# lisvulaczo/lodestar

Hardware: AMD Instinct MI355X
Metric: BLS signature sets verified/sec (whole node) at 1/2/4/8 MI355X; p50 batch latency (higher is better)
Workload: dtype u32

## Files before the change

### include/lodestar_bls.h

```cpp
#ifndef LODESTAR_BLS_H
#define LODESTAR_BLS_H

#include <stddef.h>
#include <stdint.h>

#ifdef __cplusplus
extern "C" {
#endif

#define LSG_OK 0
#define LSG_ERR_INVALID_ARG 1
#define LSG_ERR_NO_DEVICE 2
#define LSG_ERR_DEVICE 3
#define LSG_ERR_NOMEM 4
#define LSG_ERR_CLOSED 5
#define LSG_ERR_BUSY 6
#define LSG_ERR_ENTROPY 7

#define LSG_BLST_SUCCESS 0
#define LSG_BLST_BAD_ENCODING 1
#define LSG_BLST_POINT_NOT_ON_CURVE 2
#define LSG_BLST_POINT_NOT_IN_GROUP 3
#define LSG_BLST_AGGR_TYPE_MISMATCH 4
#define LSG_BLST_VERIFY_FAIL 5
// ... 144 lines not shown
int lsg_verify_deposits(lsg_ctx* ctx, const uint8_t* data184, size_t n, const uint8_t* domain32, uint64_t seed,
                        uint8_t* valid, int32_t* err);

int lsg_sign(lsg_ctx* ctx, const uint8_t* sks32, const uint8_t* msgs, uint32_t msg_len, size_t n, uint8_t* out96);
int lsg_sk_to_pk(lsg_ctx* ctx, const uint8_t* sks32, size_t n, uint8_t* out96);

int lsg_check_fp2_mul(lsg_ctx* ctx, const uint32_t* in, size_t n, uint32_t* out);
int lsg_check_fp_sqr(lsg_ctx* ctx, const uint32_t* in, size_t n, uint32_t* out);
int lsg_check_fp2_sqr(lsg_ctx* ctx, const uint32_t* in, size_t n, uint32_t* out);
int lsg_check_sums(lsg_ctx* ctx, const uint32_t* in, size_t n, uint32_t* out);
int lsg_check_fp2_lanes(lsg_ctx* ctx, const uint32_t* in, size_t n, uint32_t* out);
int lsg_check_g2_lanes(lsg_ctx* ctx, const uint32_t* in, size_t n, uint32_t* out);
int lsg_check_mf_lanes(lsg_ctx* ctx, const uint32_t* in, size_t n, uint32_t* out);
int lsg_check_pow_lanes(lsg_ctx* ctx, int32_t id, const uint32_t* in, size_t n, uint32_t* out);
int lsg_check_pow_pair(lsg_ctx* ctx, int32_t id, const uint32_t* in, size_t n, uint32_t* out);
int lsg_check_canon(lsg_ctx* ctx, const uint32_t* in, size_t n, const uint8_t* bytes48, size_t nb, uint32_t* out,
                    uint32_t* out_limbs);
int lsg_check_fp2_roots(lsg_ctx* ctx, const uint32_t* in, size_t n, uint32_t* out);
int lsg_check_batch_inv(lsg_ctx* ctx, const uint32_t* in, size_t n, uint32_t* out);
int lsg_check_map_uniform(lsg_ctx* ctx, const uint8_t* ub256, size_t n, uint8_t* out192);
int lsg_check_batch_partial_rnd(lsg_ctx* ctx, const lsg_set* sets, size_t n_sets,
                                const uint64_t* rnd , uint8_t* out576,
                                int32_t* set_err, int32_t* any_error);

int lsg_probe_fp_mul_rate(lsg_ctx* ctx, double* fp_mul_per_s, double* mad_per_s);

int lsg_probe_mad_peak(lsg_ctx* ctx, double* mad_per_s);

int lsg_last_kernel_times(lsg_ctx* ctx, const char** names, double* ms, int max);

// ... 5 lines not shown
```

### lodestar_amd/_native.py

```python
import ctypes
import os
import struct
import threading

HERE = os.path.dirname(os.path.abspath(__file__))
LIB_PATH = os.environ.get("LSG_LIB", os.path.join(HERE, "liblodestar_bls.so"))
AB_LIB_PATH = os.path.join(HERE, "liblodestar_bls_ab.so")

LSG_OK = 0
LSG_ERR_INVALID_ARG = 1
LSG_ERR_NO_DEVICE = 2
LSG_ERR_BUSY = 6
LSG_ERR_ENTROPY = 7

LSG_INVALID = 0
LSG_VALID = 1
LSG_ERROR = 2

LSG_JOB_BATCHABLE = 1
LSG_JOB_PRIORITY = 2
LSG_JOB_VALIDATE_KEYS = 4

BLST_NAMES = {
    0: "BLST_SUCCESS", 1: "BLST_BAD_ENCODING", 2: "BLST_POINT_NOT_ON_CURVE", 3: "BLST_POINT_NOT_IN_GROUP",
# ... 145 lines not shown
_lib_lock = threading.Lock()

EXPORTS = [
    "lsg_init", "lsg_init_devices", "lsg_destroy", "lsg_device_count", "lsg_last_error", "lsg_device_name",
    "lsg_reserve", "lsg_allocation_count", "lsg_verify_jobs", "lsg_verify_sets",
    "lsg_aggregate_pubkeys", "lsg_hash_to_g2", "lsg_sig_decode", "lsg_batch_partial", "lsg_final_verify",
    "lsg_probe_fp_mul_rate", "lsg_last_kernel_times", "lsg_sign", "lsg_sk_to_pk",
    "lsg_submit_jobs", "lsg_wait_jobs", "lsg_wait_jobs_node", "lsg_jobs_partial", "lsg_assign_jobs", "lsg_poll",
    "lsg_final_submit", "lsg_final_wait", "lsg_pipeline_slots", "lsg_probe_mad_peak",
    "lsg_pubkey_table_set", "lsg_pubkey_table_size", "lsg_pubkey_validate",
    "lsg_final_submit_groups", "lsg_final_wait_groups", "lsg_aggregate_signatures",
    "lsg_signing_roots", "lsg_attestation_signing_roots", "lsg_jobs_partial_device", "lsg_final_submit_device",
    "lsg_set_coalesce", "lsg_aggregate_pubkeys_multi", "lsg_check_fp2_mul",
    "lsg_check_fp_sqr", "lsg_check_fp2_sqr", "lsg_check_sums", "lsg_check_fp2_lanes", "lsg_check_g2_lanes", "lsg_check_mf_lanes",
    "lsg_check_canon", "lsg_check_fp2_roots", "lsg_check_batch_inv", "lsg_check_map_uniform",
    "lsg_check_batch_partial_rnd", "lsg_check_pow_lanes", "lsg_check_pow_pair",
    "lsg_deposit_signing_roots", "lsg_verify_deposits",
    "lsg_committees_set", "lsg_committees_clear", "lsg_committee_count",
    "lsg_object_signing_roots", "lsg_object_signing_roots_var",
    "lsg_submit_jobs_grouped", "lsg_wait_jobs_grouped",
    "lsg_msg_cache_set", "lsg_msg_cache_clear", "lsg_msg_cache_get_stats",
]


def load_library(path=LIB_PATH):
    global _lib
    with _lib_lock:
        if _lib is not None and path == LIB_PATH:
            return _lib
        if not os.path.exists(path):
            raise NativeUnavailable(f"{path} not built (run python -c 'import __graft_entry__; __graft_entry__.build()')")
# ... 56 lines not shown
        lib.lsg_aggregate_signatures.argtypes = [vp, ctypes.c_char_p, u32, ctypes.POINTER(u32), sz,
                                                 ctypes.c_char_p, pi32]
        lib.lsg_final_submit.argtypes = [vp, ctypes.c_char_p, sz, pu64]
        lib.lsg_final_wait.argtypes = [vp, u64, pi32]
        lib.lsg_pipeline_slots.argtypes = [vp, pi32]
        lib.lsg_set_coalesce.argtypes = [vp, u32, i32]
        lib.lsg_check_fp2_mul.argtypes = [vp, ctypes.c_char_p, sz, ctypes.c_char_p]
        lib.lsg_check_fp_sqr.argtypes = [vp, ctypes.c_char_p, sz, ctypes.c_char_p]
        lib.lsg_check_fp2_sqr.argtypes = [vp, ctypes.c_char_p, sz, ctypes.c_char_p]
        lib.lsg_check_sums.argtypes = [vp, ctypes.c_char_p, sz, ctypes.c_char_p]
        lib.lsg_check_fp2_lanes.argtypes = [vp, ctypes.c_char_p, sz, ctypes.c_char_p]
        lib.lsg_check_g2_lanes.argtypes = [vp, ctypes.c_char_p, sz, ctypes.c_char_p]
        lib.lsg_check_mf_lanes.argtypes = [vp, ctypes.c_char_p, sz, ctypes.c_char_p]
        lib.lsg_check_pow_lanes.argtypes = [vp, i32, ctypes.c_char_p, sz, ctypes.c_char_p]
        lib.lsg_check_pow_pair.argtypes = [vp, i32, ctypes.c_char_p, sz, ctypes.c_char_p]
        lib.lsg_check_canon.argtypes = [vp, ctypes.c_char_p, sz, ctypes.c_char_p, sz, ctypes.c_char_p, ctypes.c_char_p]
        lib.lsg_check_fp2_roots.argtypes = [vp, ctypes.c_char_p, sz, ctypes.c_char_p]
        lib.lsg_check_batch_inv.argtypes = [vp, ctypes.c_char_p, sz, ctypes.c_char_p]
        lib.lsg_check_map_uniform.argtypes = [vp, ctypes.c_char_p, sz, ctypes.c_char_p]
        lib.lsg_check_batch_partial_rnd.argtypes = [vp, ctypes.POINTER(LsgSet), sz, ctypes.POINTER(u64),
                                                    ctypes.c_char_p, pi32, pi32]
        lib.lsg_probe_mad_peak.argtypes = [vp, ctypes.POINTER(ctypes.c_double)]
        for name in EXPORTS:
            if name != "lsg_last_error":
                getattr(lib, name).restype = ctypes.c_int
        if path == LIB_PATH:
            _lib = lib
        return lib


# ... 549 lines not shown
    def check_g2_lanes(self, words):
        return self._check_lanes("lsg_check_g2_lanes", words)

    def check_mf_lanes(self, words):
        return self._check_lanes("lsg_check_mf_lanes", words)

    def check_pow(self, pow_id, words, lanes=True):
        n = len(words) // 14
        assert len(words) == 14 * n
        fn = "lsg_check_pow_lanes" if lanes else "lsg_check_pow_pair"
        out = ctypes.create_string_buffer(4 * 14 * max(n, 1))
        src = struct.pack(f"<{len(words)}I", *words)
        self._check(getattr(self.lib, fn)(self.h, pow_id, src, n, out), fn)
        return list(struct.unpack(f"<{14 * n}I", out.raw[:4 * 14 * n]))

    def check_canon(self, words, strings=()):
        n, nb = len(words) // 14, len(strings)
        assert len(words) == 14 * n and all(len(b) == 48 for b in strings)
        out = ctypes.create_string_buffer(4 * 54 * max(n, 1))
        limbs = ctypes.create_string_buffer(4 * 14 * max(nb, 1))
        src = struct.pack(f"<{len(words)}I", *words)
        self._check(self.lib.lsg_check_canon(self.h, src, n, b"".join(strings), nb, out, limbs), "lsg_check_canon")
        return (list(struct.unpack(f"<{54 * n}I", out.raw[:4 * 54 * n])),
                list(struct.unpack(f"<{14 * nb}I", limbs.raw[:4 * 14 * nb])))

    def check_fp2_roots(self, words):
        n = len(words) // 28
        assert len(words) == 28 * n
        out = ctypes.create_string_buffer(4 * 58 * n)
        src = struct.pack(f"<{len(words)}I", *words)
# ... 38 lines not shown
```

### lodestar_amd/csrc/lsg_ab.h

```cpp
#pragma once
#include <stdlib.h>

#define LSG_POW_LANES_DEFAULT 1
#define LSG_POW_LANES_MIN_DEFAULT 65536

#ifdef LSG_AB
static inline long lsg_ab_long(const char* name, long dflt) {
  const char* e = getenv(name);
  return e ? atol(e) : dflt;
}
#else
#define lsg_ab_long(name, dflt) ((long)(dflt))
#endif
```

### lodestar_amd/csrc/lsg_curve.hpp

```cpp
#pragma once
#include "lsg_tower.hpp"

LSG_INL fp_t fadd(const fp_t& a, const fp_t& b) { return fp_add(a, b); }
LSG_INL fp2_t fadd(const fp2_t& a, const fp2_t& b) { return fp2_add(a, b); }
LSG_INL fp_t fsub(const fp_t& a, const fp_t& b) { return fp_sub(a, b); }
LSG_INL fp2_t fsub(const fp2_t& a, const fp2_t& b) { return fp2_sub(a, b); }
LSG_INL fp_t fmul(const fp_t& a, const fp_t& b) { return fp_mul(a, b); }
LSG_INL fp2_t fmul(const fp2_t& a, const fp2_t& b) { return fp2_mul(a, b); }
LSG_INL fp_t fsqr(const fp_t& a) { return fp_sqr(a); }
LSG_INL fp2_t fsqr(const fp2_t& a) { return fp2_sqr(a); }
LSG_INL fp_t fneg(const fp_t& a) { return fp_neg(a); }
LSG_INL fp2_t fneg(const fp2_t& a) { return fp2_neg(a); }
LSG_INL fps_t<1, 0> fsum(const fp_t& a) { return fps(a); }
LSG_INL fp2s_t<1, 0> fsum(const fp2_t& a) { return fp2s(a); }
template <int K, int P, int N>
LSG_INL fps_t<K * P, K * N> fsum_mulk(const fps_t<P, N>& a) { return fps_mulk<K>(a); }
template <int K, int P0, int N0, int P1, int N1>
LSG_INL fp2s_t<K * P0, K * N0, K * P1, K * N1> fsum_mulk(const fp2s_t<P0, N0, P1, N1>& a) { return fp2s_mulk<K>(a); }
template <int K> LSG_INL fp_t fmulk(const fp_t& a) { return fp_mulk<K>(a); }
template <int K> LSG_INL fp2_t fmulk(const fp2_t& a) { return fp2_mulk<K>(a); }
template <class F> LSG_INL F fsub2(const F& a, const F& b, const F& c) { return (fsum(a) - b - c).carry(); }
LSG_INL fp_t fmul_b3(const fp_t& a) { return fp_mul12(a); }
LSG_INL fp2_t fmul_b3(const fp2_t& a) { return fp2_mul_b3(a); }
template <int P0, int N0, int P1, int N1>
// ... 174 lines not shown
#endif
LSG_INL const g2p_t& g2_to_pair(const g2p_t& p) { return p; }
template <class F> struct g2_layout;
template <> struct g2_layout<fp2_t> {
  static LSG_INL g2a_t in(const g2a_t& a) { return a; }
};
#ifdef LSG_FP2_LANES
template <> struct g2_layout<fp2v_t> {
  static LSG_INL g2va_t in(const g2a_t& a) { return g2v_from_pair(a); }
};
typedef fp2v_t chain_fp2_t;
#else
typedef fp2_t chain_fp2_t;
#endif

template <class F>
struct jac_t {
  F X, Y, Z;
};

template <class F>
LSG_INL jac_t<F> jac_from_proj(const proj_t<F>& p) {
  F zz = fsqr(p.Z);
  jac_t<F> r;
  bool inf = fis_zero(p.Z);
  r.X = fselect(inf, fone<F>(), fmul(p.X, p.Z));
  r.Y = fselect(inf, fone<F>(), fmul(p.Y, zz));
  r.Z = p.Z;
  return r;
}
// ... 374 lines not shown
```

### lodestar_amd/csrc/lsg_host.hip

```cpp
#include <hip/hip_runtime.h>
#include <rccl/rccl.h>
#include <stdio.h>
#include <stdlib.h>
#include <errno.h>
#include <string.h>
#include <sys/random.h>
#include <time.h>

#include <algorithm>
#include <atomic>
#include <condition_variable>
#include <chrono>
#include <mutex>
#include <shared_mutex>
#include <thread>
#include <unordered_map>
#include <string>
#include <vector>

#include "../../include/lodestar_bls.h"
#include "lsg_launch.h"
#include "lsg_layout.h"
#include "lsg_slp.h"
#include "lsg_ab.h"
// ... 473 lines not shown
}

bool agg_tree_on() { return lsg_ab_long("LSG_AGG_TREE", 0) != 0; }

Switches read_switches() {
  Switches w;
  w.package_group = lsg_ab_long("LSG_PACKAGE_GROUP", 1) != 0;
  w.sub_groups = lsg_ab_long("LSG_SUB_GROUPS", 1) != 0;
  w.nb_merge = lsg_ab_long("LSG_NB_MERGE", 1) != 0;
  w.msg_agg = lsg_ab_long("LSG_MSG_AGG", 1) != 0;
  w.msm_min_group = (size_t)std::max(1L, lsg_ab_long("LSG_MSM_MIN_GROUP", 256));
  w.b0_min = (size_t)std::max(0L, lsg_ab_long("LSG_B0_MIN", 64));
  w.b0_run = (size_t)std::max(2L, lsg_ab_long("LSG_B0_RUN", 4));
  w.seg_fold_wide = (int)lsg_ab_long("LSG_SEG_FOLD_WIDE", SEG_FOLD_WIDE);
  w.slp_items = slp_items_max();
  return w;
}
SegPlan slot_seg(Slot* s, int op, const std::vector<int32_t>& seg_off, const std::vector<int32_t>& seg_len, bool has_idx,
                 size_t idx_off, int32_t dst_base) {
  return plan_seg(s->plan, op, seg_off, seg_len, has_idx, idx_off, dst_base,
                  (int)lsg_ab_long("LSG_SEG_FOLD_WIDE", SEG_FOLD_WIDE));
}

void binv_sizes(size_t n, size_t* lv, size_t* iv);
size_t binv_lv_words(size_t n) {
  size_t a, b;
  binv_sizes(n, &a, &b);
  return a;
}
size_t binv_iv_words(size_t n) {
// ... 361 lines not shown
                                                P_<uint8_t>(s->d_hinf), P_<int32_t>(s->d_seterr), P_<uint32_t>(s->d_H),
                                                fall));
    else
      KL(s, "k_miller_fused_pair",
         lsgk::miller_fused(S_(s), ni, items, items + ni, P_<uint32_t>(s->d_P), P_<uint8_t>(s->d_pinf),
                            P_<uint8_t>(s->d_hinf), P_<int32_t>(s->d_seterr), P_<uint32_t>(s->d_H), fall, true));
    return LSG_OK;
  }
  KL(s, "k_miller_accum",
     lsgk::miller_accum(S_(s), s->K, ni, items, items + ni, P_<uint32_t>(s->d_P), P_<uint8_t>(s->d_pinf),
                        P_<uint8_t>(s->d_hinf), P_<int32_t>(s->d_seterr), (int)s->n_sets, P_<uint32_t>(s->d_lines),
                        fall));
  return LSG_OK;
}

int launch_phase(Slot* s, const PhasePlan& Ph, const uint32_t* rs, uint32_t* fall, bool export_blobs,
                 const uint32_t* rs_msm = nullptr) {
  if (!rs_msm) rs_msm = rs;
  const size_t ng = Ph.groups.size();
  if (ng == 0) return LSG_OK;
  LSG_RC(size_state(s, s->n_sets, s->n_pks, ng, Ph.n_msm, 2));
  s->cur = 1;
  if (Ph.n_msm) {
    LSG_RC(run_seg(s, 1, "msm_buckets", Ph.buckets, rs_msm, P_<uint32_t>(s->d_bkt)));
    LSG_RC(run_seg(s, 1, "msm_bits", Ph.bits, P_<uint32_t>(s->d_bkt), P_<uint32_t>(s->d_bits)));
    KL(s, "k_g2p_to_canon", lsgk::g2p_to_canon(S_(s), (int)(MSM_BITS * Ph.n_msm), P_<uint32_t>(s->d_bits),
                                               P_<uint8_t>(s->d_Sb)));
    KL(s, "slp_horner_miller",
       lsg_slp_horner_miller(S_(s), (int)Ph.n_msm, P_<uint8_t>(s->d_Sb), P_<uint8_t>(s->d_fgb)));
  }
  if (Ph.n_msm < ng) {
    const int nsm = (int)(ng - Ph.n_msm);
    LSG_RC(run_seg(s, 1, "sig_sums", Ph.sums, rs, P_<uint32_t>(s->d_S)));
    uint8_t* sb = P_<uint8_t>(s->d_Sb) + (size_t)288 * MSM_BITS * Ph.n_msm;
    KL(s, "k_g2p_to_canon", lsgk::g2p_to_canon(S_(s), nsm, P_<uint32_t>(s->d_S) + W_G2P * Ph.n_msm, sb));
    KL(s, "slp_miller_neg_g1",
       lsg_slp_miller_neg_g1(S_(s), nsm, sb, P_<uint8_t>(s->d_fgb) + 576 * Ph.n_msm));
  }
  KL(s, "k_blobs_to_fp12", lsgk::blobs_to_fp12(S_(s), (int)ng, P_<uint8_t>(s->d_fgb), fall + W_F12 * Ph.term_base));
// ... 410 lines not shown
  }
  LSG_RC(upload_plan(s));
  const uint64_t th2 = trace_host() ? now_ns() : 0;
  LSG_RC(launch_set_stages(s, &s->pkagg, A, P_<uint32_t>(s->d_fall)));
  const uint64_t th3 = trace_host() ? now_ns() : 0;
  s->rs_raw.assign(s->n_sets, 0);
  for (size_t g = 0; g < A.n_msm; g++) memset(s->rs_raw.data() + A.groups[g].first, 1, A.groups[g].len);
  if (!A.groups.empty()) {
    const bool any_small = A.n_msm < A.groups.size();
    std::vector<uint8_t> mode;
    if (any_small && A.n_msm) {
      mode.assign(s->n_sets, 0);
      for (size_t g = A.n_msm; g < A.groups.size(); g++)
        memset(mode.data() + A.groups[g].first, 1, A.groups[g].len);
    }
    LSG_RC(launch_sig_prep(s, any_small, mode.empty() ? nullptr : &mode, P_<uint32_t>(s->d_rs)));
  }
  LSG_RC(launch_phase(s, A, P_<uint32_t>(s->d_rs), P_<uint32_t>(s->d_fall), true));
  if (A.groups.empty() || s->gp.big_g < 0) {
    s->cur = 0;
    LSG_HIP(s, hipMemcpyAsync(P_<uint8_t>(s->d_gath) + 576 * LSG_MAX_DEVICES, fp12_one_blob(), 576,
                              hipMemcpyHostToDevice, s->st[0]));
    LSG_HIP(s, hipEventRecord(s->ev_part, s->st[0]));
  }
  const uint64_t th4 = trace_host() ? now_ns() : 0;
  if (s->grp_n) {
    s->cur = 1;
    LSG_RC(run_sig_groups(s, nullptr));
    s->cur = 0;
  }
  s->phA_node = node;
// ... 2205 lines not shown
    KL(s, "k_fp_pow_lanes", lsgk::fp_pow_lanes(S_(s), (int)n, id, P_<uint32_t>(s->d_aux), P_<uint32_t>(s->d_Fb)));
  else
    KL(s, "k_check_pow_pair", lsgk::check_pow_pair(S_(s), (int)n, id, P_<uint32_t>(s->d_aux), P_<uint32_t>(s->d_Fb)));
  LSG_HIP(s, hipMemcpyAsync(out, s->d_Fb.p, 4 * W_FP * n, hipMemcpyDeviceToHost, s->st[0]));
  LSG_HIP(s, hipStreamSynchronize(s->st[0]));
  keep_times(s);
  return LSG_OK;
}
int lsg_check_pow_lanes(lsg_ctx* c, int32_t id, const uint32_t* in, size_t n, uint32_t* out) {
  return check_pow(c, id, in, n, out, true);
}
int lsg_check_pow_pair(lsg_ctx* c, int32_t id, const uint32_t* in, size_t n, uint32_t* out) {
  return check_pow(c, id, in, n, out, false);
}

int lsg_check_canon(lsg_ctx* c, const uint32_t* in, size_t n, const uint8_t* bytes48, size_t nb, uint32_t* out,
                    uint32_t* out_limbs) {
  constexpr size_t WOUT = lsgk::CHECK_CANON_OUT;
  if (!c || (n && (!in || !out)) || (nb && (!bytes48 || !out_limbs)) || n > 0x7fffffffull / (4 * WOUT) ||
      nb > 0x7fffffffull / (4 * W_FP))
    return LSG_ERR_INVALID_ARG;
  LSG_ENTER(c);
  Slot* s = &c->dev[0]->util;
  timer_reset(s);
  if (n) {
    LSG_RC(ensure(s, s->d_aux, 4 * W_FP * n));
    LSG_RC(ensure(s, s->d_Fb, 4 * WOUT * n));
    LSG_HIP(s, hipMemcpyAsync(s->d_aux.p, in, 4 * W_FP * n, hipMemcpyHostToDevice, s->st[0]));
    KL(s, "k_check_canon", lsgk::check_canon(S_(s), (int)n, P_<uint32_t>(s->d_aux), P_<uint32_t>(s->d_Fb)));
    LSG_HIP(s, hipMemcpyAsync(out, s->d_Fb.p, 4 * WOUT * n, hipMemcpyDeviceToHost, s->st[0]));
// ... 141 lines not shown
```

### lodestar_amd/csrc/lsg_k_sig.hip

```cpp
#include "lsg_kcommon.hpp"

__global__ void LSG_KERNEL_ATTR k_sig_decode(int n, const uint8_t* __restrict__ sig, const uint32_t* __restrict__ sig_len,
                                             uint32_t* __restrict__ sig_aff, uint8_t* __restrict__ inf,
                                             int32_t* __restrict__ err) {
  LANE_ITEM(n);
  uint32_t len = sig_len[item];
  g2a_t p;
  p.x = fp2_zero();
  p.y = fp2_zero();
  bool is_inf = false;
  int e;
  if (len == 96)
    e = g2_uncompress(p, is_inf, sig + 192 * item);
  else if (len == 192)
    e = g2_deserialize_uncompressed(p, is_inf, sig + 192 * item);
  else
    e = LSG_BLST_INVALID_SIZE;
  lane_store(sig_aff, item, p);
  if (lead) {
    inf[item] = is_inf ? 1 : 0;
    err[item] = e;
  }
}

// ... 145 lines not shown
      const bool cur_use = use;
      if (k + ips < len) use = fetch(k + ips);
      if (cur_use) acc = proj_is_inf(acc) ? proj_from_aff(cur) : g2_add_mixed(acc, cur);
    }
  }
#pragma unroll 1
  for (int o = ips >> 1; o >= 1; o >>= 1) acc = g2_add(acc, shfl_xor_t(acc, LSG_GROUP * o));
  if (active && j == 0) {
    if (out >= 0)
      lane_store(dst, (size_t)out, acc);
    else
      lane_store(tmp, (size_t)(-out - 1), acc);
  }
}

__global__ void LSG_KERNEL_ATTR k_g2a_to_bytes(int n, const uint32_t* __restrict__ pts, const uint8_t* __restrict__ inf,
                                               uint8_t* __restrict__ out) {
  LANE_ITEM(n);
  (void)lead;
  g2_serialize(out + 192 * item, lane_load<g2a_t>(pts, item), inf[item] != 0);
}

__global__ void LSG_KERNEL_ATTR k_g2p_compress(int n, const uint32_t* __restrict__ pts, uint8_t* __restrict__ out96) {
  LANE_ITEM(n);
  (void)lead;
  g2p_t p = lane_load<g2p_t>(pts, item);
  bool is_inf = proj_is_inf(p);
  g2a_t a;
  if (is_inf) {
    a.x = fp2_zero();
// ... 72 lines not shown
    hipLaunchKernelGGL(k_sig_proj, dim3(lane_blocks((size_t)n)), dim3(LSG_TPB), 0, st, n, sig_aff, inf, err, pinf, out);
    hipError_t e = hipGetLastError();
    if (e != hipSuccess || !rnd) return e;
  }
  return sig_scale_only(st, n, sig_aff, inf, err, pinf, rnd, mode, out);
}
hipError_t sig_scale_only(hipStream_t st, int n, const uint32_t* sig_aff, const uint8_t* inf, const int32_t* err,
                          const uint8_t* pinf, const uint64_t* rnd, const uint8_t* mode, uint32_t* out) {
  LSG_LAUNCH_ITEMS(k_sig_scale3, n, st, n, sig_aff, inf, err, pinf, rnd, mode, out);
}
hipError_t sig_agg_seg(hipStream_t st, int n_chunks, int ips_log2, const int32_t* chunks, const int32_t* gather,
                       const uint32_t* sig_aff, const uint8_t* inf, const int32_t* err, uint32_t* dst, uint32_t* tmp) {
  LSG_LAUNCH_ITEMS(k_sig_agg_seg, (size_t)n_chunks << ips_log2, st, n_chunks, ips_log2, chunks, gather, sig_aff, inf, err,
                   dst, tmp);
}
hipError_t g2a_to_bytes(hipStream_t st, int n, const uint32_t* pts, const uint8_t* inf, uint8_t* out192) {
  LSG_LAUNCH_ITEMS(k_g2a_to_bytes, n, st, n, pts, inf, out192);
}
hipError_t g2p_compress(hipStream_t st, int n, const uint32_t* pts, uint8_t* out96) {
  LSG_LAUNCH_ITEMS(k_g2p_compress, n, st, n, pts, out96);
}
hipError_t g2p_to_canon(hipStream_t st, int n, const uint32_t* pts, uint8_t* out288) {
  LSG_LAUNCH_ITEMS(k_g2p_to_canon, n, st, n, pts, out288);
}
hipError_t sign(hipStream_t st, int n, const uint8_t* sks, const uint32_t* H, uint8_t* out96) {
  LSG_LAUNCH_ITEMS(k_sign, n, st, n, sks, H, out96);
}
}
```

### lodestar_amd/csrc/lsg_launch.h

```cpp
#pragma once
#include <hip/hip_runtime.h>
#include <stddef.h>
#include <stdint.h>

constexpr uint32_t LSG_MC_ROW = 0x80000000u;

namespace lsgk {
struct PowLanes {
  int min_items = 0;
  uint32_t* state = nullptr;
  uint32_t* pa = nullptr;
  uint32_t* pb = nullptr;
  bool on(int items) const { return min_items > 0 && items >= min_items && state && pa && pb; }
};
constexpr size_t POW_SIG_STATE = 4 * 14 + 2, POW_MAP_STATE = 10 * 14;
hipError_t expand_msg(hipStream_t st, int n, const uint8_t* msg, const uint32_t* off, const uint32_t* len,
                      const uint8_t* dst, uint32_t dst_len, uint8_t* ub);
hipError_t h2c_prep(hipStream_t st, int n, const uint8_t* ub, uint32_t* U, uint32_t* norms);
hipError_t h2c_map(hipStream_t st, int n, const uint32_t* U, const uint32_t* ninv, uint32_t* Hp,
                   const PowLanes& pw = PowLanes());
hipError_t h2c_clear(hipStream_t st, int n, uint32_t* Hp, uint32_t* zN, uint8_t* hinf, bool pair_form = false);
hipError_t h2c_gather(hipStream_t st, int n, const uint32_t* mid, const uint32_t* Hm, const uint8_t* hinfm, uint32_t* H,
                      uint8_t* hinf);
hipError_t h2c_affine(hipStream_t st, int n, const uint32_t* Hp, const uint32_t* ninv, const uint8_t* hinf,
// ... 12 lines not shown
hipError_t object_signing_root(hipStream_t st, int n, const uint8_t* objs, uint32_t obj_len, const uint8_t* domains,
                               uint32_t dstride, uint8_t* out32);
hipError_t msg_roots(hipStream_t st, int n, uint8_t* msg, const uint32_t* off, uint32_t* len);
hipError_t msg_roots_var(hipStream_t st, int n, uint8_t* msg, const uint32_t* off, uint32_t* len, uint8_t* out32);

hipError_t sig_decode(hipStream_t st, int n, const uint8_t* sig, const uint32_t* sig_len, uint32_t* sig_aff,
                      uint8_t* inf, int32_t* err, const PowLanes& pw = PowLanes());
hipError_t sig_subgroup(hipStream_t st, int n, const uint32_t* sig_aff, const uint8_t* inf, int32_t* err,
                        bool pair_form = false);
hipError_t sig_prep(hipStream_t st, int n, const uint32_t* sig_aff, const uint8_t* inf, const int32_t* err,
                    const uint8_t* pinf, const uint64_t* rnd, const uint8_t* mode, uint32_t* out);
hipError_t sig_scale_only(hipStream_t st, int n, const uint32_t* sig_aff, const uint8_t* inf, const int32_t* err,
                          const uint8_t* pinf, const uint64_t* rnd, const uint8_t* mode, uint32_t* out);
hipError_t sig_agg_seg(hipStream_t st, int n_chunks, int ips_log2, const int32_t* chunks, const int32_t* gather,
                       const uint32_t* sig_aff, const uint8_t* inf, const int32_t* err, uint32_t* dst, uint32_t* tmp);
hipError_t g2a_to_bytes(hipStream_t st, int n, const uint32_t* pts, const uint8_t* inf, uint8_t* out192);
hipError_t g2p_compress(hipStream_t st, int n, const uint32_t* pts, uint8_t* out96);
hipError_t g2p_to_canon(hipStream_t st, int n, const uint32_t* pts, uint8_t* out288);
hipError_t sign(hipStream_t st, int n, const uint8_t* sks, const uint32_t* H, uint8_t* out96);

hipError_t pk_decode(hipStream_t st, int n, const uint8_t* pk, uint32_t stride, const uint32_t* pk_len, uint32_t* pts,
                     int32_t* err, const uint32_t* tab, const uint8_t* tab_ok, uint32_t tab_n);
hipError_t pk_validate(hipStream_t st, int n, const uint8_t* pk, uint32_t len, uint32_t* pts, int32_t* err);
hipError_t pk_keyvalidate(hipStream_t st, int n, const int32_t* keys, const uint8_t* pk, const uint32_t* pk_len,
                          int32_t* code);
hipError_t pk_keyvalidate_apply(hipStream_t st, int n, const int32_t* sets, const int32_t* code, int32_t* set_err);
hipError_t pk_gather_aff(hipStream_t st, int n, const uint8_t* pk, uint32_t stride, const uint32_t* pk_len, uint32_t* pts,
                         uint8_t* inf, int32_t* err, const uint32_t* tab, const uint8_t* tab_ok, uint32_t tab_n);
hipError_t pk_agg_seg(hipStream_t st, int n_chunks, int ips_log2, const int32_t* chunks, const uint8_t* pk, uint32_t stride,
                      const uint32_t* pk_len, int32_t* err, const uint32_t* tab, const uint8_t* tab_ok, uint32_t tab_n,
// ... 78 lines not shown
```

### lodestar_amd/csrc/lsg_plan.hpp

```cpp
#pragma once
#include <stddef.h>
#include <stdint.h>

#include <string.h>

#include <algorithm>
#include <functional>
#include <utility>
#include <vector>

#include "../../include/lodestar_bls.h"
#include "lsg_bits.h"
#include "lsg_ssz.hpp"

namespace lsgp {

typedef std::pair<size_t, size_t> Range;
typedef std::pair<int32_t, int32_t> ItemRange;

inline std::vector<Range> chunkify(size_t len, size_t min_per_chunk) {
  std::vector<Range> out;
  size_t chunk_count = len / min_per_chunk;
  if (chunk_count <= 1) {
    out.push_back({0, len});
// ... 32 lines not shown
constexpr int SEG_FOLD = 16;
constexpr int SEG_FOLD_FP12 = 4;
constexpr int SEG_FOLD_WIDE = 64;
constexpr size_t SEG_WIDE_PAIRS = 131072;

struct Switches {
  bool package_group = true;
  bool sub_groups = true;
  bool nb_merge = true;
  bool msg_agg = true;
  size_t msm_min_group = 256;
  size_t b0_min = 64;
  size_t b0_run = 4;
  int seg_fold_wide = SEG_FOLD_WIDE;
  size_t slp_items = 2048;
};

inline int ips_for(double avg, int32_t max_len, int fold) {
  int l = 0;
  while (l < 5 && ((int32_t)(fold << l) < max_len || (double)(2 << l) * 4.0 <= avg)) l++;
  return l;
}

inline SegPlan plan_seg(std::vector<int32_t>& A, int op, const std::vector<int32_t>& seg_off,
                        const std::vector<int32_t>& seg_len, bool has_idx, size_t idx_off, int32_t dst_base,
                        int fold_wide) {
  SegPlan P;
  P.op = op;
  P.has_idx = has_idx;
  P.idx_off = idx_off;
  const size_t ns = seg_len.size();
  if (ns == 0) return P;
  size_t total = 0;
  for (int32_t l : seg_len) total += (size_t)l;
  struct Pend {
    int32_t seg, off, len;
  };
  std::vector<Pend> cur(ns);
  for (size_t s = 0; s < ns; s++) cur[s] = {(int32_t)s, seg_off[s], seg_len[s]};
  double avg = (double)total / (double)ns;
  int src = 0, tmp_out = 1;
  while (!cur.empty()) {
    SegPass pass;
    int32_t max_len = 0;
    for (const Pend& p : cur) max_len = std::max(max_len, p.len);
    int fold = op == 2 ? SEG_FOLD_FP12 : SEG_FOLD;
    pass.ips_log2 = ips_for(avg, max_len, fold);
    if (op != 2 && (cur.size() << 5) >= SEG_WIDE_PAIRS) {
      int l = 0;
      while (l < pass.ips_log2 && (int32_t)(fold_wide << l) < max_len) l++;
      pass.ips_log2 = l;
      fold = fold_wide;
    }
    pass.src = src;
    pass.tmp_out = tmp_out;
    const int32_t cap = (int32_t)((1 << pass.ips_log2) * fold);
    pass.chunk_off = A.size();
    std::vector<Pend> nxt;
    int32_t t = 0;
    size_t nxt_total = 0;
    for (const Pend& p : cur) {
      if (p.len <= cap) {
        A.push_back(p.off);
        A.push_back(p.len);
        A.push_back(dst_base + p.seg);
        pass.n_chunks++;
      } else {
        const int32_t first = t;
        for (int32_t o = 0; o < p.len; o += cap) {
          A.push_back(p.off + o);
          A.push_back(std::min(cap, p.len - o));
          A.push_back(-(t + 1));
          t++;
          pass.n_chunks++;
        }
        nxt.push_back({p.seg, first, t - first});
        nxt_total += (size_t)(t - first);
      }
    }
    P.tmp_items = std::max(P.tmp_items, (size_t)t);
    P.passes.push_back(pass);
    avg = nxt.empty() ? 1.0 : (double)nxt_total / (double)nxt.size();
    cur.swap(nxt);
    src = tmp_out;
    tmp_out = tmp_out == 1 ? 2 : 1;
  }
  return P;
}

struct Grp {
  size_t first = 0, len = 0;
  bool msm = false;
};

inline SegPlan plan_msg_lists(std::vector<int32_t>& A, const uint32_t* msg_id, size_t n_msgs, const Grp& g,
                              int fold_wide) {
  std::vector<int32_t> cnt(n_msgs, 0), off(n_msgs), fill;
  for (size_t i = g.first; i < g.first + g.len; i++) cnt[msg_id[i]]++;
  int32_t tot = 0;
  for (size_t j = 0; j < n_msgs; j++) {
    off[j] = tot;
    tot += cnt[j];
// ... 76 lines not shown
    const size_t idx_off = A.size();
    A.resize(idx_off + (size_t)tot);
    int32_t* idx = A.data() + idx_off;
    std::vector<int32_t> fill(seg_off);
    for (size_t g = 0; g < Ph.n_msm; g++) {
      const int c = cw[g], nw = 64 / c;
      const uint64_t dm = (1ull << c) - 1;
      for (size_t i = Ph.groups[g].first; i < Ph.groups[g].first + Ph.groups[g].len; i++) {
        const uint64_t r = rnd[i];
        for (int w = 0; w < nw; w++) {
          const uint32_t d = (uint32_t)((r >> (c * w)) & dm);
          if (d) idx[fill[bucket(g, w, d)]++] = (int32_t)i;
        }
      }
    }
    Ph.buckets = plan_seg(A, 1, seg_off, seg_len, true, idx_off, 0, sw.seg_fold_wide);
    const size_t bidx = A.size();
    std::vector<int32_t> boff, blen;
    for (size_t g = 0; g < Ph.n_msm; g++) {
      const int c = cw[g], nw = 64 / c;
      for (int w = 0; w < nw; w++)
        for (int j = 0; j < c; j++) {
          boff.push_back((int32_t)(A.size() - bidx));
          for (uint32_t d = 1; d < (1u << c); d++)
            if ((d >> j) & 1u) A.push_back((int32_t)bucket(g, w, d));
          blen.push_back((int32_t)(A.size() - bidx) - boff.back());
        }
    }
    Ph.bits = plan_seg(A, 1, boff, blen, true, bidx, 0, sw.seg_fold_wide);
  }
  if (Ph.n_msm < ng) {
// ... 953 lines not shown
```

Measured before the change: 4.020 million.

## Fuse signature prep into MSM bucket accumulation with cost-model chunk planning

Adds a kernel that accumulates MSM buckets directly from affine signatures using mixed additions, gathering and checking usability inline. This removes the separate sig_prep pass and its intermediate projective buffer when no small groups exist. The bucket plan now picks items-per-segment with a host-side cost model and sorts first-pass chunks by length to balance waves. The trade-off is extra host planning work and a more complex launch path, plus a new check entry point for validating the kernel.

```diff
diff --git a/include/lodestar_bls.h b/include/lodestar_bls.h
--- a/include/lodestar_bls.h
+++ b/include/lodestar_bls.h
@@ -182,6 +182,10 @@
 int lsg_check_mf_lanes(lsg_ctx* ctx, const uint32_t* in, size_t n, uint32_t* out);
 int lsg_check_pow_lanes(lsg_ctx* ctx, int32_t id, const uint32_t* in, size_t n, uint32_t* out);
 int lsg_check_pow_pair(lsg_ctx* ctx, int32_t id, const uint32_t* in, size_t n, uint32_t* out);
+int lsg_check_msm_buckets(lsg_ctx* ctx, int32_t mode, const uint8_t* sigs96, size_t n, const int32_t* err,
+                          const uint8_t* inf, const uint8_t* pinf, const int32_t* idx, size_t n_idx,
+                          const int32_t* chunks, size_t n_chunks, int32_t ips_log2, const int32_t* chunks2,
+                          size_t n_chunks2, int32_t ips_log2_2, size_t n_tmp, size_t n_out, uint8_t* out96);
 int lsg_check_canon(lsg_ctx* ctx, const uint32_t* in, size_t n, const uint8_t* bytes48, size_t nb, uint32_t* out,
                     uint32_t* out_limbs);
 int lsg_check_fp2_roots(lsg_ctx* ctx, const uint32_t* in, size_t n, uint32_t* out);
diff --git a/lodestar_amd/_native.py b/lodestar_amd/_native.py
--- a/lodestar_amd/_native.py
+++ b/lodestar_amd/_native.py
@@ -183,7 +183,7 @@
     "lsg_set_coalesce", "lsg_aggregate_pubkeys_multi", "lsg_check_fp2_mul",
     "lsg_check_fp_sqr", "lsg_check_fp2_sqr", "lsg_check_sums", "lsg_check_fp2_lanes", "lsg_check_g2_lanes", "lsg_check_mf_lanes",
     "lsg_check_canon", "lsg_check_fp2_roots", "lsg_check_batch_inv", "lsg_check_map_uniform",
-    "lsg_check_batch_partial_rnd", "lsg_check_pow_lanes", "lsg_check_pow_pair",
+    "lsg_check_batch_partial_rnd", "lsg_check_pow_lanes", "lsg_check_pow_pair", "lsg_check_msm_buckets",
     "lsg_deposit_signing_roots", "lsg_verify_deposits",
     "lsg_committees_set", "lsg_committees_clear", "lsg_committee_count",
     "lsg_object_signing_roots", "lsg_object_signing_roots_var",
@@ -270,6 +270,9 @@
         lib.lsg_check_mf_lanes.argtypes = [vp, ctypes.c_char_p, sz, ctypes.c_char_p]
         lib.lsg_check_pow_lanes.argtypes = [vp, i32, ctypes.c_char_p, sz, ctypes.c_char_p]
         lib.lsg_check_pow_pair.argtypes = [vp, i32, ctypes.c_char_p, sz, ctypes.c_char_p]
+        lib.lsg_check_msm_buckets.argtypes = [vp, i32, ctypes.c_char_p, sz, ctypes.c_char_p, ctypes.c_char_p,
+                                              ctypes.c_char_p, ctypes.c_char_p, sz, ctypes.c_char_p, sz, i32,
+                                              ctypes.c_char_p, sz, i32, sz, sz, ctypes.c_char_p]
         lib.lsg_check_canon.argtypes = [vp, ctypes.c_char_p, sz, ctypes.c_char_p, sz, ctypes.c_char_p, ctypes.c_char_p]
         lib.lsg_check_fp2_roots.argtypes = [vp, ctypes.c_char_p, sz, ctypes.c_char_p]
         lib.lsg_check_batch_inv.argtypes = [vp, ctypes.c_char_p, sz, ctypes.c_char_p]
@@ -849,6 +852,20 @@
         self._check(getattr(self.lib, fn)(self.h, pow_id, src, n, out), fn)
         return list(struct.unpack(f"<{14 * n}I", out.raw[:4 * 14 * n]))
 
+    def check_msm_buckets(self, mode, sigs, err, inf, pinf, idx, chunks, ips_log2, n_out, chunks2=(), ips_log2_2=0,
+                          n_tmp=0):
+        n = len(sigs)
+        assert len(err) == len(inf) == len(pinf) == n and all(len(b) == 96 for b in sigs)
+        flat = [v for t in chunks for v in t]
+        flat2 = [v for t in chunks2 for v in t]
+        out = ctypes.create_string_buffer(96 * max(n_out, 1))
+        rc = self.lib.lsg_check_msm_buckets(
+            self.h, mode, b"".join(sigs), n, struct.pack(f"<{n}i", *err), bytes(inf), bytes(pinf),
+            struct.pack(f"<{len(idx)}i", *idx), len(idx), struct.pack(f"<{len(flat)}i", *flat), len(chunks), ips_log2,
+            struct.pack(f"<{len(flat2)}i", *flat2), len(chunks2), ips_log2_2, n_tmp, n_out, out)
+        self._check(rc, "lsg_check_msm_buckets")
+        return [out.raw[96 * k:96 * k + 96] for k in range(n_out)]
+
     def check_canon(self, words, strings=()):
         n, nb = len(words) // 14, len(strings)
         assert len(words) == 14 * n and all(len(b) == 48 for b in strings)
diff --git a/lodestar_amd/csrc/lsg_ab.h b/lodestar_amd/csrc/lsg_ab.h
--- a/lodestar_amd/csrc/lsg_ab.h
+++ b/lodestar_amd/csrc/lsg_ab.h
@@ -3,6 +3,9 @@
 
 #define LSG_POW_LANES_DEFAULT 1
 #define LSG_POW_LANES_MIN_DEFAULT 65536
+
+#define LSG_MSM_FOLD_DEFAULT 1
+#define LSG_MSM_IPS_DEFAULT (-1)
 
 #ifdef LSG_AB
 static inline long lsg_ab_long(const char* name, long dflt) {
diff --git a/lodestar_amd/csrc/lsg_curve.hpp b/lodestar_amd/csrc/lsg_curve.hpp
--- a/lodestar_amd/csrc/lsg_curve.hpp
+++ b/lodestar_amd/csrc/lsg_curve.hpp
@@ -212,6 +212,28 @@
 typedef fp2_t chain_fp2_t;
 #endif
 
+template <class F, class FETCH>
+LSG_INL proj_t<F> g2_fold_mixed(int first, int step, int len, FETCH&& fetch) {
+  proj_t<F> acc = proj_inf<F>();
+  bool any = false, use = false;
+  g2a_t a;
+  a.x = fzero<fp2_t>();
+  a.y = fzero<fp2_t>();
+  if (first < len) use = fetch(first, a);
+#pragma unroll 1
+  for (int k = first; k < len; k += step) {
+    const g2a_t cur = a;
+    const bool cur_use = use;
+    if (k + step < len) use = fetch(k + step, a);
+    if (cur_use) {
+      const aff_t<F> q = g2_layout<F>::in(cur);
+      acc = any ? gadd(acc, q) : proj_from_aff(q);
+      any = true;
+    }
+  }
+  return acc;
+}
+
 template <class F>
 struct jac_t {
   F X, Y, Z;
diff --git a/lodestar_amd/csrc/lsg_host.hip b/lodestar_amd/csrc/lsg_host.hip
--- a/lodestar_amd/csrc/lsg_host.hip
+++ b/lodestar_amd/csrc/lsg_host.hip
@@ -511,6 +511,8 @@
   w.b0_run = (size_t)std::max(2L, lsg_ab_long("LSG_B0_RUN", 4));
   w.seg_fold_wide = (int)lsg_ab_long("LSG_SEG_FOLD_WIDE", SEG_FOLD_WIDE);
   w.slp_items = slp_items_max();
+  w.msm_fold = lsg_ab_long("LSG_MSM_FOLD", LSG_MSM_FOLD_DEFAULT) != 0;
+  w.msm_ips = (int)std::max(-1L, std::min(lsg_ab_long("LSG_MSM_IPS", LSG_MSM_IPS_DEFAULT), 5L));
   return w;
 }
 SegPlan slot_seg(Slot* s, int op, const std::vector<int32_t>& seg_off, const std::vector<int32_t>& seg_len, bool has_idx,
@@ -902,6 +904,24 @@
   return LSG_OK;
 }
 
+int run_msm_buckets(Slot* s, const SegPlan& P, const uint32_t* rs_msm, uint32_t* dst) {
+  if (!s->sw.msm_fold) return run_seg(s, 1, "msm_buckets", P, rs_msm, dst);
+  LSG_RC(size_seg(s, 1, P));
+  uint32_t* tmp[3] = {nullptr, P_<uint32_t>(s->seg_tmp[1][0]), P_<uint32_t>(s->seg_tmp[1][1])};
+  for (size_t k = 0; k < P.passes.size(); k++) {
+    const SegPass& q = P.passes[k];
+    if (k == 0)
+      KL(s, "msm_buckets", lsgk::msm_bucket_seg(S_(s), q.n_chunks, q.ips_log2, PL(s, q.chunk_off), PL(s, P.idx_off),
+                                                P_<uint32_t>(s->d_sigaff), P_<uint8_t>(s->d_siginf),
+                                                P_<int32_t>(s->d_seterr), P_<uint8_t>(s->d_pinf), dst, tmp[q.tmp_out],
+                                                !fp2_lanes_on()));
+    else
+      KL(s, "msm_buckets", lsgk::seg_reduce(S_(s), 1, q.n_chunks, q.ips_log2, PL(s, q.chunk_off), nullptr, tmp[q.src],
+                                            dst, tmp[q.tmp_out]));
+  }
+  return LSG_OK;
+}
+
 int launch_phase(Slot* s, const PhasePlan& Ph, const uint32_t* rs, uint32_t* fall, bool export_blobs,
                  const uint32_t* rs_msm = nullptr) {
   if (!rs_msm) rs_msm = rs;
@@ -910,7 +930,7 @@
   LSG_RC(size_state(s, s->n_sets, s->n_pks, ng, Ph.n_msm, 2));
   s->cur = 1;
   if (Ph.n_msm) {
-    LSG_RC(run_seg(s, 1, "msm_buckets", Ph.buckets, rs_msm, P_<uint32_t>(s->d_bkt)));
+    LSG_RC(run_msm_buckets(s, Ph.buckets, rs_msm, P_<uint32_t>(s->d_bkt)));
     LSG_RC(run_seg(s, 1, "msm_bits", Ph.bits, P_<uint32_t>(s->d_bkt), P_<uint32_t>(s->d_bits)));
     KL(s, "k_g2p_to_canon", lsgk::g2p_to_canon(S_(s), (int)(MSM_BITS * Ph.n_msm), P_<uint32_t>(s->d_bits),
                                                P_<uint8_t>(s->d_Sb)));
@@ -1351,7 +1371,8 @@
       for (size_t g = A.n_msm; g < A.groups.size(); g++)
         memset(mode.data() + A.groups[g].first, 1, A.groups[g].len);
     }
-    LSG_RC(launch_sig_prep(s, any_small, mode.empty() ? nullptr : &mode, P_<uint32_t>(s->d_rs)));
+    if (any_small || !s->sw.msm_fold)
+      LSG_RC(launch_sig_prep(s, any_small, mode.empty() ? nullptr : &mode, P_<uint32_t>(s->d_rs)));
   }
   LSG_RC(launch_phase(s, A, P_<uint32_t>(s->d_rs), P_<uint32_t>(s->d_fall), true));
   if (A.groups.empty() || s->gp.big_g < 0) {
@@ -3587,6 +3608,75 @@
   return check_pow(c, id, in, n, out, false);
 }
 
+int lsg_check_msm_buckets(lsg_ctx* c, int32_t mode, const uint8_t* sigs96, size_t n, const int32_t* err,
+                          const uint8_t* inf, const uint8_t* pinf, const int32_t* idx, size_t n_idx,
+                          const int32_t* chunks, size_t n_chunks, int32_t ips_log2, const int32_t* chunks2,
+                          size_t n_chunks2, int32_t ips_log2_2, size_t n_tmp, size_t n_out, uint8_t* out96) {
+  const size_t lim = (size_t)1 << 20;
+  if (!c || mode < 0 || mode > 2 || !sigs96 || !err || !inf || !pinf || !chunks || !out96 || (n_idx && !idx) ||
+      (n_chunks2 && !chunks2) || n == 0 || n > lim || n_idx > lim || n_chunks == 0 || n_chunks > lim || n_chunks2 > lim ||
+      n_tmp > lim || n_out == 0 || n_out > lim || ips_log2 < 0 || ips_log2 > 5 || ips_log2_2 < 0 || ips_log2_2 > 5)
+    return LSG_ERR_INVALID_ARG;
+  for (size_t k = 0; k < n_idx; k++)
+    if (idx[k] < 0 || (size_t)idx[k] >= n) return LSG_ERR_INVALID_ARG;
+  std::vector<uint8_t> tmp_set(n_tmp, 0), out_set(n_out, 0);
+  auto mark = [&](int32_t out, bool tmp_ok) {
+    std::vector<uint8_t>& v = out >= 0 ? out_set : tmp_set;
+    const size_t o = out >= 0 ? (size_t)out : (size_t)(-(int64_t)out - 1);
+    if ((out < 0 && !tmp_ok) || o >= v.size() || v[o]) return false;
+    v[o] = 1;
+    return true;
+  };
+  for (size_t k = 0; k < n_chunks; k++) {
+    const int32_t off = chunks[3 * k], len = chunks[3 * k + 1];
+    if (off < 0 || len < 0 || (size_t)off + (size_t)len > n_idx || !mark(chunks[3 * k + 2], true)) return LSG_ERR_INVALID_ARG;
+  }
+  for (size_t k = 0; k < n_chunks2; k++) {
+    const int32_t off = chunks2[3 * k], len = chunks2[3 * k + 1];
+    if (off < 0 || len < 0 || (size_t)off + (size_t)len > n_tmp || !mark(chunks2[3 * k + 2], false)) return LSG_ERR_INVALID_ARG;
+  }
+  for (uint8_t v : tmp_set)
+    if (!v) return LSG_ERR_INVALID_ARG;
+  for (uint8_t v : out_set)
+    if (!v) return LSG_ERR_INVALID_ARG;
+  LSG_ENTER(c);
+  timer_reset(&c->dev[0]->util);
+  Slot* s;
+  LSG_RC(sig_decode_impl(c, sigs96, 96, n, false, &s));
+  LSG_HIP(s, hipMemcpyAsync(s->d_seterr.p, err, 4 * n, hipMemcpyHostToDevice, s->st[0]));
+  LSG_HIP(s, hipMemcpyAsync(s->d_siginf.p, inf, n, hipMemcpyHostToDevice, s->st[0]));
+  LSG_HIP(s, hipMemcpyAsync(s->d_pinf.p, pinf, n, hipMemcpyHostToDevice, s->st[0]));
+  s->plan.assign(idx, idx + n_idx);
+  const size_t c1 = s->plan.size();
+  s->plan.insert(s->plan.end(), chunks, chunks + 3 * n_chunks);
+  const size_t c2 = s->plan.size();
+  if (n_chunks2) s->plan.insert(s->plan.end(), chunks2, chunks2 + 3 * n_chunks2);
+  LSG_RC(upload_plan(s));
+  LSG_RC(ensure(s, s->d_bkt, 4 * W_G2P * n_out));
+  LSG_RC(ensure(s, s->seg_tmp[1][0], 4 * W_G2P * std::max(n_tmp, (size_t)1)));
+  LSG_RC(ensure(s, s->d_aux, 96 * n_out));
+  uint32_t* dst = P_<uint32_t>(s->d_bkt);
+  uint32_t* tmp = P_<uint32_t>(s->seg_tmp[1][0]);
+  if (mode == 2) {
+    KL(s, "k_sig_prep", lsgk::sig_prep(S_(s), (int)n, P_<uint32_t>(s->d_sigaff), P_<uint8_t>(s->d_siginf),
+                                       P_<int32_t>(s->d_seterr), P_<uint8_t>(s->d_pinf), nullptr, nullptr,
+                                       P_<uint32_t>(s->d_rs)));
+    KL(s, "msm_buckets", lsgk::seg_reduce(S_(s), 1, (int)n_chunks, ips_log2, PL(s, c1), PL(s, 0), P_<uint32_t>(s->d_rs),
+                                          dst, tmp));
+  } else {
+    KL(s, "msm_buckets", lsgk::msm_bucket_seg(S_(s), (int)n_chunks, ips_log2, PL(s, c1), PL(s, 0),
+                                              P_<uint32_t>(s->d_sigaff), P_<uint8_t>(s->d_siginf),
+                                              P_<int32_t>(s->d_seterr), P_<uint8_t>(s->d_pinf), dst, tmp, mode == 1));
+  }
+  if (n_chunks2)
+    KL(s, "msm_buckets", lsgk::seg_reduce(S_(s), 1, (int)n_chunks2, ips_log2_2, PL(s, c2), nullptr, tmp, dst, nullptr));
+  KL(s, "k_g2p_compress", lsgk::g2p_compress(S_(s), (int)n_out, dst, P_<uint8_t>(s->d_aux)));
+  LSG_HIP(s, hipMemcpyAsync(out96, s->d_aux.p, 96 * n_out, hipMemcpyDeviceToHost, s->st[0]));
+  LSG_HIP(s, hipStreamSynchronize(s->st[0]));
+  keep_times(s);
+  return LSG_OK;
+}
+
 int lsg_check_canon(lsg_ctx* c, const uint32_t* in, size_t n, const uint8_t* bytes48, size_t nb, uint32_t* out,
                     uint32_t* out_limbs) {
   constexpr size_t WOUT = lsgk::CHECK_CANON_OUT;
diff --git a/lodestar_amd/csrc/lsg_k_sig.hip b/lodestar_amd/csrc/lsg_k_sig.hip
--- a/lodestar_amd/csrc/lsg_k_sig.hip
+++ b/lodestar_amd/csrc/lsg_k_sig.hip
@@ -183,6 +183,53 @@
   }
 }
 
+template <class F>
+LSG_DEVI void msm_bucket_item(int n_chunks, int ips_log2, const int32_t* __restrict__ chunks,
+                              const int32_t* __restrict__ gather, const uint32_t* __restrict__ sig_aff,
+                              const uint8_t* __restrict__ inf, const int32_t* __restrict__ err,
+                              const uint8_t* __restrict__ pinf, uint32_t* __restrict__ dst, uint32_t* __restrict__ tmp) {
+  lsg_lane_setup();
+  const size_t item = gtid() / LSG_GROUP;
+  const size_t c = item >> ips_log2;
+  const int ips = 1 << ips_log2, j = (int)(item & (size_t)(ips - 1));
+  const bool active = c < (size_t)n_chunks;
+  g2p_t acc = proj_inf<fp2_t>();
+  int out = 0;
+  if (active) {
+    const int off = chunks[3 * c], len = chunks[3 * c + 1];
+    out = chunks[3 * c + 2];
+    acc = g2_to_pair(g2_fold_mixed<F>(j, ips, len, [&](int k, g2a_t& a) {
+      const size_t i = (size_t)gather[off + k];
+      a = lane_load<g2a_t>(sig_aff, i);
+      return sig_usable(i, inf, err, pinf);
+    }));
+  }
+#pragma unroll 1
+  for (int o = ips >> 1; o >= 1; o >>= 1) acc = g2_add(acc, shfl_xor_t(acc, LSG_GROUP * o));
+  if (active && j == 0) {
+    if (out >= 0)
+      lane_store(dst, (size_t)out, acc);
+    else
+      lane_store(tmp, (size_t)(-out - 1), acc);
+  }
+}
+__global__ void LSG_KERNEL_ATTR k_msm_bucket_seg(int n_chunks, int ips_log2, const int32_t* __restrict__ chunks,
+                                                 const int32_t* __restrict__ gather, const uint32_t* __restrict__ sig_aff,
+                                                 const uint8_t* __restrict__ inf, const int32_t* __restrict__ err,
+                                                 const uint8_t* __restrict__ pinf, uint32_t* __restrict__ dst,
+                                                 uint32_t* __restrict__ tmp) {
+  msm_bucket_item<chain_fp2_t>(n_chunks, ips_log2, chunks, gather, sig_aff, inf, err, pinf, dst, tmp);
+}
+#ifdef LSG_FP2_LANES
+__global__ void LSG_KERNEL_ATTR k_msm_bucket_seg_pair(int n_chunks, int ips_log2, const int32_t* __restrict__ chunks,
+                                                      const int32_t* __restrict__ gather,
+                                                      const uint32_t* __restrict__ sig_aff, const uint8_t* __restrict__ inf,
+                                                      const int32_t* __restrict__ err, const uint8_t* __restrict__ pinf,
+                                                      uint32_t* __restrict__ dst, uint32_t* __restrict__ tmp) {
+  msm_bucket_item<fp2_t>(n_chunks, ips_log2, chunks, gather, sig_aff, inf, err, pinf, dst, tmp);
+}
+#endif
+
 __global__ void LSG_KERNEL_ATTR k_g2a_to_bytes(int n, const uint32_t* __restrict__ pts, const uint8_t* __restrict__ inf,
                                                uint8_t* __restrict__ out) {
   LANE_ITEM(n);
@@ -285,6 +332,18 @@
   LSG_LAUNCH_ITEMS(k_sig_agg_seg, (size_t)n_chunks << ips_log2, st, n_chunks, ips_log2, chunks, gather, sig_aff, inf, err,
                    dst, tmp);
 }
+hipError_t msm_bucket_seg(hipStream_t st, int n_chunks, int ips_log2, const int32_t* chunks, const int32_t* gather,
+                          const uint32_t* sig_aff, const uint8_t* inf, const int32_t* err, const uint8_t* pinf,
+                          uint32_t* dst, uint32_t* tmp, bool pair_form) {
+#ifdef LSG_FP2_LANES
+  if (pair_form)
+    LSG_LAUNCH_ITEMS(k_msm_bucket_seg_pair, (size_t)n_chunks << ips_log2, st, n_chunks, ips_log2, chunks, gather, sig_aff,
+                     inf, err, pinf, dst, tmp);
+#endif
+  (void)pair_form;
+  LSG_LAUNCH_ITEMS(k_msm_bucket_seg, (size_t)n_chunks << ips_log2, st, n_chunks, ips_log2, chunks, gather, sig_aff, inf,
+                   err, pinf, dst, tmp);
+}
 hipError_t g2a_to_bytes(hipStream_t st, int n, const uint32_t* pts, const uint8_t* inf, uint8_t* out192) {
   LSG_LAUNCH_ITEMS(k_g2a_to_bytes, n, st, n, pts, inf, out192);
 }
diff --git a/lodestar_amd/csrc/lsg_launch.h b/lodestar_amd/csrc/lsg_launch.h
--- a/lodestar_amd/csrc/lsg_launch.h
+++ b/lodestar_amd/csrc/lsg_launch.h
@@ -50,6 +50,9 @@
                           const uint8_t* pinf, const uint64_t* rnd, const uint8_t* mode, uint32_t* out);
 hipError_t sig_agg_seg(hipStream_t st, int n_chunks, int ips_log2, const int32_t* chunks, const int32_t* gather,
                        const uint32_t* sig_aff, const uint8_t* inf, const int32_t* err, uint32_t* dst, uint32_t* tmp);
+hipError_t msm_bucket_seg(hipStream_t st, int n_chunks, int ips_log2, const int32_t* chunks, const int32_t* gather,
+                          const uint32_t* sig_aff, const uint8_t* inf, const int32_t* err, const uint8_t* pinf,
+                          uint32_t* dst, uint32_t* tmp, bool pair_form = false);
 hipError_t g2a_to_bytes(hipStream_t st, int n, const uint32_t* pts, const uint8_t* inf, uint8_t* out192);
 hipError_t g2p_compress(hipStream_t st, int n, const uint32_t* pts, uint8_t* out96);
 hipError_t g2p_to_canon(hipStream_t st, int n, const uint32_t* pts, uint8_t* out288);
diff --git a/lodestar_amd/csrc/lsg_plan.hpp b/lodestar_amd/csrc/lsg_plan.hpp
--- a/lodestar_amd/csrc/lsg_plan.hpp
+++ b/lodestar_amd/csrc/lsg_plan.hpp
@@ -70,6 +70,8 @@
   size_t b0_run = 4;
   int seg_fold_wide = SEG_FOLD_WIDE;
   size_t slp_items = 2048;
+  bool msm_fold = true;
+  int msm_ips = -1;
 };
 
 inline int ips_for(double avg, int32_t max_len, int fold) {
@@ -78,9 +80,23 @@
   return l;
 }
 
+inline void sort_chunks_desc(int32_t* chunks, size_t n) {
+  struct Tri {
+    int32_t off, len, out;
+  };
+  std::vector<Tri> v(n);
+  for (size_t c = 0; c < n; c++) v[c] = {chunks[3 * c], chunks[3 * c + 1], chunks[3 * c + 2]};
+  std::stable_sort(v.begin(), v.end(), [](const Tri& a, const Tri& b) { return a.len > b.len; });
+  for (size_t c = 0; c < n; c++) {
+    chunks[3 * c] = v[c].off;
+    chunks[3 * c + 1] = v[c].len;
+    chunks[3 * c + 2] = v[c].out;
+  }
+}
+
 inline SegPlan plan_seg(std::vector<int32_t>& A, int op, const std::vector<int32_t>& seg_off,
                         const std::vector<int32_t>& seg_len, bool has_idx, size_t idx_off, int32_t dst_base,
-                        int fold_wide) {
+                        int fold_wide, int first_ips = -1) {
   SegPlan P;
   P.op = op;
   P.has_idx = has_idx;
@@ -108,6 +124,11 @@
       pass.ips_log2 = l;
       fold = fold_wide;
     }
+    const bool first_given = first_ips >= 0 && P.passes.empty();
+    if (first_given) {
+      pass.ips_log2 = std::min(first_ips, 5);
+      fold = std::max(SEG_FOLD, fold_wide);
+    }
     pass.src = src;
     pass.tmp_out = tmp_out;
     const int32_t cap = (int32_t)((1 << pass.ips_log2) * fold);
@@ -134,6 +155,7 @@
         nxt_total += (size_t)(t - first);
       }
     }
+    if (first_given) sort_chunks_desc(A.data() + pass.chunk_off, (size_t)pass.n_chunks);
     P.tmp_items = std::max(P.tmp_items, (size_t)t);
     P.passes.push_back(pass);
     avg = nxt.empty() ? 1.0 : (double)nxt_total / (double)nxt.size();
@@ -142,6 +164,103 @@
     tmp_out = tmp_out == 1 ? 2 : 1;
   }
   return P;
+}
+
+struct SegCost {
+  size_t adds = 0, waves = 0;
+  int chain = 0;
+  int passes = 0;
+};
+inline SegCost bucket_cost(const std::vector<int32_t>& lens, int first_ips, int fold_wide) {
+  SegCost c;
+  std::vector<int32_t> split, nxt;
+  const std::vector<int32_t>* cur = &lens;
+  size_t total = 0;
+  for (int32_t l : lens) total += (size_t)l;
+  double avg = lens.empty() ? 1.0 : (double)total / (double)lens.size();
+  while (!cur->empty()) {
+    int32_t max_len = 0;
+    for (int32_t l : *cur) max_len = std::max(max_len, l);
+    int fold = SEG_FOLD, l2 = ips_for(avg, max_len, fold);
+    if ((cur->size() << 5) >= SEG_WIDE_PAIRS) {
+      int l = 0;
+      while (l < l2 && (int32_t)(fold_wide << l) < max_len) l++;
+      l2 = l;
+      fold = fold_wide;
+    }
+    const bool given = first_ips >= 0 && c.passes == 0;
+    if (given) {
+      l2 = std::min(first_ips, 5);
+      fold = std::max(SEG_FOLD, fold_wide);
+    }
+    const int32_t cap = (int32_t)(fold << l2), ips = 1 << l2;
+    const std::vector<int32_t>* chunks = cur;
+    std::vector<int32_t> pieces;
+    if (max_len > cap) {
+      split.clear();
+      size_t nt = 0;
+      for (int32_t l : *cur) {
+        if (l <= cap) {
+          split.push_back(l);
+          continue;
+        }
+        for (int32_t o = 0; o < l; o += cap) split.push_back(std::min(cap, l - o));
+        pieces.push_back((l + cap - 1) / cap);
+        nt += (size_t)pieces.back();
+      }
+      if (given) std::sort(split.begin(), split.end(), std::greater<int32_t>());
+      chunks = &split;
+      avg = pieces.empty() ? 1.0 : (double)nt / (double)pieces.size();
+    }
+    const size_t per_wave = (size_t)32 >> l2, n = chunks->size();
+    int pass_chain = 0;
+    size_t waves = 0;
+    for (size_t w = 0; w < n; w += per_wave, waves++) {
+      int32_t longest = (*chunks)[w];
+      if (!given || chunks != &lens)
+        for (size_t k = w; k < std::min(n, w + per_wave); k++) longest = std::max(longest, (*chunks)[k]);
+      const int cost = (longest > 0 ? (int)((longest + ips - 1) / ips) - 1 : 0) + l2;
+      c.adds += (size_t)32 * (size_t)cost;
+      pass_chain = std::max(pass_chain, cost);
+    }
+    if (c.passes == 0) c.waves = waves;
+    c.chain += pass_chain;
+    c.passes++;
+    nxt.swap(pieces);
+    cur = &nxt;
+    if (nxt.empty()) break;
+  }
+  return c;
+}
+constexpr double BUCKET_COST_TOL = 1.25;
+constexpr size_t BUCKET_MIN_WAVES = 256;
+inline int bucket_ips(const std::vector<int32_t>& seg_len, int fold_wide) {
+  const int max_passes = bucket_cost(seg_len, -1, fold_wide).passes;
+  std::vector<int32_t> lens(seg_len);
+  std::sort(lens.begin(), lens.end(), std::greater<int32_t>());
+  SegCost cost[6];
+  size_t best = ~(size_t)0;
+  for (int l = 0; l <= 5; l++) {
+    cost[l] = bucket_cost(lens, l, fold_wide);
+    if (cost[l].passes <= max_passes) best = std::min(best, cost[l].adds);
+  }
+  int pick = 5;
+  for (int l = 0; l <= 5; l++)
+    if (cost[l].passes <= max_passes && (double)cost[l].adds <= BUCKET_COST_TOL * (double)best) pick = l;
+  while (pick < 5 && cost[pick].waves < BUCKET_MIN_WAVES && cost[pick].chain > SEG_FOLD &&
+         cost[pick + 1].passes == cost[pick].passes)
+    pick++;
+  return pick;
+}
+inline SegPlan plan_buckets(std::vector<int32_t>& A, const std::vector<int32_t>& seg_off,
+                            const std::vector<int32_t>& seg_len, size_t idx_off, int fold_wide, int force_ips = -1) {
+  if (force_ips < 0) {
+    int32_t max_len = 0;
+    for (int32_t l : seg_len) max_len = std::max(max_len, l);
+    if (max_len <= SEG_FOLD) return plan_seg(A, 1, seg_off, seg_len, true, idx_off, 0, fold_wide);
+  }
+  const int pick = force_ips >= 0 ? std::min(force_ips, 5) : bucket_ips(seg_len, fold_wide);
+  return plan_seg(A, 1, seg_off, seg_len, true, idx_off, 0, fold_wide, pick);
 }
 
 struct Grp {
@@ -248,7 +367,8 @@
         }
       }
     }
-    Ph.buckets = plan_seg(A, 1, seg_off, seg_len, true, idx_off, 0, sw.seg_fold_wide);
+    Ph.buckets = sw.msm_fold ? plan_buckets(A, seg_off, seg_len, idx_off, sw.seg_fold_wide, sw.msm_ips)
+                             : plan_seg(A, 1, seg_off, seg_len, true, idx_off, 0, sw.seg_fold_wide);
     const size_t bidx = A.size();
     std::vector<int32_t> boff, blen;
     for (size_t g = 0; g < Ph.n_msm; g++) {
```

After: 4.095 million, median of 6. 1.02x the previous value.
